# rafaelghiorzi/YOLO-MS

Hardware: AMD Instinct MI355X
Metric: images/sec (train+infer) YOLO-MS-S 640x640 bf16 at 1/2/4/8 MI355X; mAP parity (higher is better)
Workload: dtype bf16; 1 GPU; configs[2]: YOLO-MS-S (reference YOLOv8-'s' graph) 640x640 bf16 training, B=64/GPU, fwd+loss+bwd+SGD-nesterov step; global_batch=64, per_gpu_batch=64, img=640, parallelism=dp1, hip_graph=False

## Files before the change

include/yms.h:

```cpp
#ifndef YMS_H
#define YMS_H

#include <stddef.h>
#include <stdint.h>

#ifdef __cplusplus
extern "C" {
#endif

typedef int yms_status;
#define YMS_OK 0
#define YMS_ERR_INVALID 1
#define YMS_ERR_UNSUPPORTED 2
#define YMS_ERR_LAUNCH 3

#define YMS_F32 0
#define YMS_BF16 1
#define YMS_F16 2

#define YMS_ACT_NONE 0
#define YMS_ACT_SILU 1

typedef struct {
  int n, h, w, cin, cout, k, stride, pad, ho, wo, dtype;
// ... 56 lines not shown
  yms_conv_shape shape;
  const void* dz; int dz_ld, dz_off;
  const void* wpacked_t;
  void* dx; int dx_ld, dx_off;
  int accumulate;
} yms_conv_dgrad_job;
yms_status yms_conv_fwd_group(int njobs, const yms_conv_fwd_job* jobs, void* stream);
yms_status yms_conv_dgrad_group(int njobs, const yms_conv_dgrad_job* jobs, void* stream);
int yms_conv_fwd_group_launches(int njobs, const yms_conv_fwd_job* jobs);
int yms_conv_dgrad_group_launches(int njobs, const yms_conv_dgrad_job* jobs);
size_t yms_conv_wgrad_ws_bytes(const yms_conv_shape* s);
yms_status yms_conv_wgrad(const yms_conv_shape* s, const void* x, int x_ld, int x_off,
                          const void* dz, int dz_ld, int dz_off, float* ws, size_t ws_bytes,
                          float* dw, int accumulate, void* stream);

yms_status yms_bn_fold(int c, const float* gamma, const float* beta, const float* rmean,
                       const float* rvar, float eps, float* scale, float* shift, void* stream);
yms_status yms_bn_finalize(int c, float* stats, int rows, int stats_ld, long count,
                           const float* gamma, const float* beta, float* rmean, float* rvar,
                           float momentum, float eps, float* mean_invstd, float* scale,
                           float* shift, void* stream);
yms_status yms_bn_finalize_ld(int c, float* stats, int rows, int stats_ld, long count,
                              const float* gamma, const float* beta, float* rmean, float* rvar,
                              float momentum, float eps, float* mean_invstd, int mi_ld, float* scale,
                              float* shift, void* stream);
yms_status yms_affine_act(int dtype, long npix, int c, const void* z, int z_ld, int z_off,
                          const float* scale, const float* shift, int act,
                          const void* res, int res_ld, int res_off,
                          void* y, int y_ld, int y_off, void* stream);
int yms_bn_bwd_rows(long npix, int c);
yms_status yms_bn_act_bwd_reduce(int dtype, long npix, int c, const void* z, int z_ld, int z_off,
                                 const void* gy, int gy_ld, int gy_off, const float* scale,
                                 const float* shift, const float* mean_invstd, int act,
                                 float* ws, void* stream);
yms_status yms_bn_act_bwd_finalize(int c, const float* ws, int rows, long count,
                                   float* dgamma, float* dbeta, float* coef, void* stream);
yms_status yms_bn_act_bwd_apply(int dtype, long npix, int c, const void* z, int z_ld, int z_off,
                                const void* gy, int gy_ld, int gy_off, const float* scale,
                                const float* shift, const float* mean_invstd, const float* coef,
                                int act, void* dz, int dz_ld, int dz_off,
                                void* gres, int gres_ld, int gres_off, int gres_acc, void* stream);
yms_status yms_bn_act_bwd_reduce_finalize(int dtype, long npix, int c, const void* z, int z_ld, int z_off,
                                          const void* gy, int gy_ld, int gy_off, const float* scale,
                                          const float* shift, const float* mean_invstd, int act, float* ws,
                                          unsigned* counter, float* dgamma, float* dbeta, float* coef,
                                          void* stream);
yms_status yms_bias_bwd(int dtype, long npix, int c, const void* gy, int gy_ld, int gy_off,
                        float* ws, unsigned* counter, float* dbias, void* stream);
typedef struct {
  int c;
  float* stats; int rows, stats_ld; long count;
  const float* gamma; const float* beta; float* rmean; float* rvar;
  float momentum, eps;
  float* mean_invstd; int mi_ld;
  float* scale; float* shift;
} yms_bn_finalize_job;
typedef struct {
  long npix; int c;
  const void* z; int z_ld, z_off;
  const void* gy; int gy_ld, gy_off;
  const float* scale; const float* shift; const float* mean_invstd; const float* coef;
  int act;
  void* out; int out_ld, out_off;
  void* res; int res_ld, res_off, res_acc;
  float* ws; unsigned* counter; float* dbias;
} yms_bn_pass_job;
typedef struct {
  int c;
  const float* ws; int rows; long count;
  float* dgamma; float* dbeta; float* coef;
} yms_bn_bwd_finalize_job;
yms_status yms_bn_finalize_group(int njobs, const yms_bn_finalize_job* jobs, void* stream);
yms_status yms_affine_act_group(int dtype, int njobs, const yms_bn_pass_job* jobs, void* stream);
yms_status yms_bn_act_bwd_reduce_group(int dtype, int njobs, const yms_bn_pass_job* jobs, void* stream);
yms_status yms_bn_act_bwd_finalize_group(int njobs, const yms_bn_bwd_finalize_job* jobs, void* stream);
yms_status yms_bn_act_bwd_apply_group(int dtype, int njobs, const yms_bn_pass_job* jobs, void* stream);
yms_status yms_bias_bwd_group(int dtype, int njobs, const yms_bn_pass_job* jobs, void* stream);

yms_status yms_sppf_pool_fwd(int dtype, int n, int h, int w, int c, void* buf, int ld, int off,
                             void* stream);
size_t yms_sppf_ws_bytes(int n, int h, int w, int c);
yms_status yms_sppf_pool_bwd(int dtype, int n, int h, int w, int c, const void* buf, int ld,
                             int off, void* gbuf, int gld, int goff, void* ws, void* stream);
yms_status yms_upsample2x_fwd(int dtype, int n, int h, int w, int c, const void* x, int x_ld,
                              int x_off, void* y, int y_ld, int y_off, void* stream);
yms_status yms_upsample2x_bwd(int dtype, int n, int h, int w, int c, const void* gy, int gy_ld,
                              int gy_off, void* gx, int gx_ld, int gx_off, int accumulate,
                              void* stream);
yms_status yms_pack_input(int dtype, int n, int c, int h, int w, const float* x, void* y, int ld,
                          void* stream);
yms_status yms_nhwc_to_nchw(int dtype, int dtype_nchw, int n, int h, int w, int c, const void* x,
                            int ld, int off, void* y, void* stream);
yms_status yms_nchw_to_nhwc(int dtype_nchw, int dtype, int n, int h, int w, int c, const void* x,
                            void* y, int ld, int off, int accumulate, void* stream);
yms_status yms_zero(void* p, size_t bytes, void* stream);
yms_status yms_copy(void* dst, const void* src, size_t bytes, void* stream);
yms_status yms_cast(int dtype_in, int dtype_out, long count, const void* x, void* y, void* stream);

typedef struct {
  int n, h, w, c, k, dtype;
} yms_dw_shape;
int yms_dwconv_stats_rows(const yms_dw_shape* s);
yms_status yms_dwconv_fwd(const yms_dw_shape* s, const void* x, int x_ld, int x_off, const float* w, void* y,
                          int y_ld, int y_off, const float* scale, const float* shift, int act, float* stats,
                          int stats_ld, void* stream);
yms_status yms_dwconv_dgrad(const yms_dw_shape* s, const void* dz, int dz_ld, int dz_off, const float* w, void* dx,
                            int dx_ld, int dx_off, int accumulate, void* stream);
size_t yms_dwconv_wgrad_ws_bytes(const yms_dw_shape* s);
yms_status yms_dwconv_wgrad(const yms_dw_shape* s, const void* x, int x_ld, int x_off, const void* dz, int dz_ld,
                            int dz_off, float* ws, size_t ws_bytes, float* dw, int accumulate, void* stream);
yms_status yms_add_views(int dtype, long npix, int c, const void* a, int a_ld, int a_off, const void* b, int b_ld,
                         int b_off, void* y, int y_ld, int y_off, int accumulate, void* stream);
yms_status yms_add_grad2(int dtype, long npix, int c, const void* g, int g_ld, int g_off, void* ga, int ga_ld,
                         int ga_off, int acc1, void* gb, int gb_ld, int gb_off, int acc2, void* stream);

yms_status yms_map_match(int n_images, const float* det_boxes, const float* det_scores, const int* det_labels,
                         const int* det_off, const float* gt_boxes, const int* gt_labels, const int* gt_off,
                         uint8_t* tp, uint8_t* kept, int* rank_ws, int max_gt_per_image, void* stream);
yms_status yms_map_accumulate(int n_det, const float* scores, const int* labels, const int* image,
                              const uint8_t* tp, const uint8_t* kept, int n_classes, const int* n_gt,
                              double* ap, double* map);
yms_status yms_map_match_coco(int n_images, int n_det, const float* det_boxes, const float* det_scores,
                              const int* det_labels, const int* det_off, const float* gt_boxes, const int* gt_labels,
                              const int* gt_off, int n_thr, const double* iou_thrs, uint16_t* matched,
                              uint16_t* ignored, uint8_t* gt_ignore, int* rank_ws, int max_gt_per_image,
                              void* stream);
yms_status yms_map_accumulate_coco(int n_det, const float* scores, const int* labels, const int* image,
                                   const int* rank, const uint16_t* matched, const uint16_t* ignored, int n_thr,
                                   int n_classes, const int* npig, double* precision, double* recall);

yms_status yms_resize_normalize(int dtype, int n, const void* images, int out_h, int out_w, const float* mean,
                                const float* std, void* out, void* stream);
size_t yms_augment_image_bytes(void);
yms_status yms_augment_normalize(int dtype, int n, const void* images, int out_h, int out_w, const float* mean,
                                 const float* std, void* out, void* stream);
size_t yms_mosaic_image_bytes(void);
yms_status yms_mosaic_normalize(int dtype, int n, const void* records, int out_h, int out_w, const float* mean,
                                const float* std, void* out, void* stream);

size_t yms_det_loss_ws_bytes(int batch, int anchors, int nc, int n_targets);
yms_status yms_det_loss(int dtype, int batch, int nc, int nlevels, const void* const* maps, void* const* grads,
                        const int* hs, const int* ws_, const float* strides, int ld, const float* targets,
                        int n_targets, float img_w, float img_h, int iou_type, const float* pos_weight,
                        const float* lambdas, void* ws, size_t ws_bytes, float* out, void* stream);
yms_status yms_scale_by_device_scalar(int dtype, int nbuf, void* const* bufs, const long* counts, const float* g,
                                      void* stream);

yms_status yms_head_decode(int dtype, int n, int nc, int nlev, const void* const* lvl,
                           const int* hs, const int* ws, int no_ld, const float* strides,
                           float* out, float conf, float* boxes_xyxy, float* nms_score,
                           int* label, void* stream);
yms_status yms_dfl(int dtype, int n, int A, int ch, const void* x, void* out, void* stream);
yms_status yms_nms_prep(int n, int A, int nc, const float* pred, float conf, float* boxes_xyxy,
                        float* score, int* label, void* stream);
size_t yms_nms_ws_bytes(int n, int A, int nc);
size_t yms_nms_ws_bytes_min(int n, int A, int nc);
yms_status yms_nms_classwise(int n, int A, int nc, const float* boxes_xyxy, const float* score,
                             const int* label, double iou, int64_t* keep_idx, int* keep_lbl,
                             int* counts, void* ws, size_t ws_bytes, void* stream);
yms_status yms_nms_single(int m, const float* boxes, const float* scores, double iou,
                          int64_t* keep, int* count, void* ws, size_t ws_bytes, void* stream);

#ifdef __cplusplus
}
#endif
#endif
// ... 1 lines not shown
```

yolo-ms_amd/csrc/bn_pool.hip:

```cpp
#include <cstdlib>
#include <algorithm>
#include <vector>

#include "yms_common.hpp"

namespace yms {

static inline unsigned grid_for(long items, int block = 256, long cap = 16384) {
  long g = (items + block - 1) / block;
  if (g < 1) g = 1;
  return (unsigned)std::min(g, cap);
}

__global__ void bn_fold_kernel(int c, const float* g, const float* b, const float* rm,
                               const float* rv, float eps, float* scale, float* shift) {
  const int i = blockIdx.x * blockDim.x + threadIdx.x;
  if (i >= c) return;
  if (!g) {
    scale[i] = 1.0f;
    shift[i] = b ? b[i] : 0.0f;
    return;
  }
  const float sc = g[i] / sqrtf(rv[i] + eps);
  scale[i] = sc;
// ... 720 lines not shown
      }
    }
    Vec8<T>::store(buf + (long)pix * ld + out_off + g * 8, m);
  }
}

template <typename T>
__global__ void pool5_argmax_kernel(int n, int h, int w, int c, const T* buf, int ld, int in_off,
                                    uint8_t* arg) {
  const int G = (c + 7) >> 3;
  const uint32_t total = (uint32_t)n * h * w * G;
  for (uint32_t t = blockIdx.x * blockDim.x + threadIdx.x; t < total; t += gridDim.x * blockDim.x) {
    const int g = (int)(t % G);
    uint32_t r = t / G;
    const int x = (int)(r % w);
    r /= w;
    const int y = (int)(r % h);
    const int b = (int)(r / h);
    const int c0 = g * 8, nv = min(8, c - c0);
    float best[8];
    uint8_t idx[8];
#pragma unroll
    for (int i = 0; i < 8; ++i) { best[i] = -INFINITY; idx[i] = 255; }
    for (int ky = 0; ky < 5; ++ky) {
      const int yy = y - 2 + ky;
      if (yy < 0 || yy >= h) continue;
      for (int kx = 0; kx < 5; ++kx) {
        const int xx = x - 2 + kx;
        if (xx < 0 || xx >= w) continue;
        float v[8];
        load8(buf + (((long)b * h + yy) * w + xx) * ld + in_off + c0, nv, v);
#pragma unroll
        for (int i = 0; i < 8; ++i)
          if (idx[i] == 255 || v[i] > best[i] || v[i] != v[i]) {
            best[i] = v[i];
            idx[i] = (uint8_t)(ky * 5 + kx);
          }
      }
    }
    uint8_t* a = arg + ((((long)b * h + y) * w + x) * G + g) * 8;
#pragma unroll
    for (int i = 0; i < 8; ++i) a[i] = idx[i];
  }
}

template <typename T>
__global__ void pool5_gather_kernel(int n, int h, int w, int c, const uint8_t* arg, T* g, int ld,
                                    int in_off, int out_off) {
  const int G = (c + 7) >> 3;
  const uint32_t total = (uint32_t)n * h * w * G;
  for (uint32_t t = blockIdx.x * blockDim.x + threadIdx.x; t < total; t += gridDim.x * blockDim.x) {
    const int gg = (int)(t % G);
    uint32_t r = t / G;
    const int x = (int)(r % w);
    r /= w;
    const int y = (int)(r % h);
    const int b = (int)(r / h);
    const int c0 = gg * 8, nv = min(8, c - c0);
    float acc[8];
    load8(g + (((long)b * h + y) * w + x) * ld + in_off + c0, nv, acc);
    for (int ky = 0; ky < 5; ++ky) {
      const int oy = y - ky + 2;
      if (oy < 0 || oy >= h) continue;
      for (int kx = 0; kx < 5; ++kx) {
        const int ox = x - kx + 2;
        if (ox < 0 || ox >= w) continue;
        const long o = ((long)b * h + oy) * w + ox;
        const uint8_t* a = arg + (o * G + gg) * 8;
        const uint2 av = *reinterpret_cast<const uint2*>(a);
        const uint8_t want = (uint8_t)(ky * 5 + kx);
        float gv[8];
        load8(g + o * ld + out_off + c0, nv, gv);
#pragma unroll
        for (int i = 0; i < 8; ++i) {
          const uint8_t ai = (uint8_t)(((i < 4 ? av.x : av.y) >> (8 * (i & 3))) & 0xff);
          if (ai == want) acc[i] += gv[i];
        }
      }
    }
    store8(g + (((long)b * h + y) * w + x) * ld + in_off + c0, nv, acc);
  }
}


template <typename T>
__global__ void upsample_fwd_kernel(int n, int h, int w, int c, const T* x, int x_ld, int x_off,
                                    T* y, int y_ld, int y_off) {
  const int G = (c + 7) >> 3;
  const int H2 = 2 * h, W2 = 2 * w;
  const long total = (long)n * H2 * W2 * G;
  for (long t = blockIdx.x * (long)blockDim.x + threadIdx.x; t < total; t += (long)gridDim.x * blockDim.x) {
    const int g = (int)(t % G);
    long r = t / G;
    const int X = (int)(r % W2);
    r /= W2;
    const int Y = (int)(r % H2);
    const int b = (int)(r / H2);
    const int c0 = g * 8, nv = min(8, c - c0);
    float v[8];
    load8(x + (((long)b * h + (Y >> 1)) * w + (X >> 1)) * x_ld + x_off + c0, nv, v);
    store8(y + (((long)b * H2 + Y) * W2 + X) * y_ld + y_off + c0, nv, v);
  }
}

template <typename T>
__global__ void upsample_bwd_kernel(int n, int h, int w, int c, const T* gy, int gy_ld, int gy_off,
                                    T* gx, int gx_ld, int gx_off, int accumulate) {
  const int G = (c + 7) >> 3;
  const int W2 = 2 * w;
  const long total = (long)n * h * w * G;
  for (long t = blockIdx.x * (long)blockDim.x + threadIdx.x; t < total; t += (long)gridDim.x * blockDim.x) {
    const int g = (int)(t % G);
    long r = t / G;
    const int x = (int)(r % w);
    r /= w;
    const int y = (int)(r % h);
    const int b = (int)(r / h);
    const int c0 = g * 8, nv = min(8, c - c0);
    float s[8];
    T* dst = gx + (((long)b * h + y) * w + x) * gx_ld + gx_off + c0;
    if (accumulate) load8(dst, nv, s);
    else {
#pragma unroll
      for (int i = 0; i < 8; ++i) s[i] = 0.f;
    }
#pragma unroll
    for (int d = 0; d < 4; ++d) {
      float v[8];
      const int Y = 2 * y + (d >> 1), X = 2 * x + (d & 1);
      load8(gy + (((long)b * 2 * h + Y) * W2 + X) * gy_ld + gy_off + c0, nv, v);
#pragma unroll
      for (int i = 0; i < 8; ++i) s[i] += v[i];
    }
    store8(dst, nv, s);
  }
}

template <typename T>
__global__ void pack_input_kernel(int n, int c, int h, int w, const float* x, T* y, int ld) {
  const long npix = (long)n * h * w;
  const long hw = (long)h * w;
  for (long t = blockIdx.x * (long)blockDim.x + threadIdx.x; t < npix; t += (long)gridDim.x * blockDim.x) {
    const long b = t / hw, s = t - b * hw;
    for (int c0 = 0; c0 < ld; c0 += 8) {
      float v[8];
#pragma unroll
      for (int i = 0; i < 8; ++i) v[i] = (c0 + i < c) ? x[(b * c + c0 + i) * hw + s] : 0.0f;
      Vec8<T>::store(y + t * ld + c0, v);
    }
  }
}

template <typename TI, typename TO>
__global__ void nhwc_to_nchw_kernel(int n, long hw, int c, const TI* x, int ld, int off, TO* y) {
  __shared__ float tile[64][65];
  const long pt = (long)blockIdx.x * 64;
  const int ct = blockIdx.y * 64;
  const int b = blockIdx.z;
  const int tx = threadIdx.x & 63, ty = threadIdx.x >> 6;
  for (int r = ty; r < 64; r += 4) {
    const long p = pt + r;
    const int ch = ct + tx;
    tile[r][tx] = (p < hw && ch < c) ? (float)x[((long)b * hw + p) * ld + off + ch] : 0.f;
  }
  __syncthreads();
  for (int r = ty; r < 64; r += 4) {
// ... 319 lines not shown
                            mean_invstd, c, scale, shift, stream);
}

yms_status yms_affine_act(int dtype, long npix, int c, const void* z, int z_ld, int z_off,
                          const float* scale, const float* shift, int act,
                          const void* res, int res_ld, int res_off,
                          void* y, int y_ld, int y_off, void* stream) {
  const yms_bn_pass_job j{npix, c, z, z_ld, z_off, nullptr, 0, 0, scale, shift, nullptr, nullptr, act, y, y_ld, y_off,
                          (void*)res, res_ld, res_off};
  return run_pass<AffinePass>(dtype, 1, &j, stream);
}

int yms_bn_bwd_rows(long npix, int c) {
  if (npix <= 0 || c <= 0) return 0;
  return (int)pix_blocks(npix, bwd_pix_per_block(npix, c, false));
}

yms_status yms_bn_act_bwd_reduce(int dtype, long npix, int c, const void* z, int z_ld, int z_off,
                                 const void* gy, int gy_ld, int gy_off, const float* scale,
                                 const float* shift, const float* mean_invstd, int act,
                                 float* ws, void* stream) {
  const yms_bn_pass_job j{npix, c, z, z_ld, z_off, gy, gy_ld, gy_off, scale, shift, mean_invstd, nullptr, act,
                          nullptr, 0, 0, nullptr, 0, 0, 0, ws};
  return run_pass<ReducePass>(dtype, 1, &j, stream);
}

yms_status yms_bn_act_bwd_finalize(int c, const float* ws, int rows, long count, float* dgamma,
                                   float* dbeta, float* coef, void* stream) {
  const yms_bn_bwd_finalize_job j{c, ws, rows, count, dgamma, dbeta, coef};
  return run_pass<BwdFinalizePass>(0, 1, &j, stream);
}

yms_status yms_bn_act_bwd_apply(int dtype, long npix, int c, const void* z, int z_ld, int z_off,
                                const void* gy, int gy_ld, int gy_off, const float* scale,
                                const float* shift, const float* mean_invstd, const float* coef,
                                int act, void* dz, int dz_ld, int dz_off,
                                void* gres, int gres_ld, int gres_off, int gres_acc, void* stream) {
  const yms_bn_pass_job j{npix, c, z, z_ld, z_off, gy, gy_ld, gy_off, scale, shift, mean_invstd, coef, act,
                          dz, dz_ld, dz_off, gres, gres_ld, gres_off, gres_acc};
  return run_pass<ApplyPass>(dtype, 1, &j, stream);
}

yms_status yms_bn_act_bwd_reduce_finalize(int dtype, long npix, int c, const void* z, int z_ld, int z_off,
                                          const void* gy, int gy_ld, int gy_off, const float* scale,
                                          const float* shift, const float* mean_invstd, int act, float* ws,
                                          unsigned* counter, float* dgamma, float* dbeta, float* coef,
                                          void* stream) {
  const yms_bn_pass_job j{npix, c, z, z_ld, z_off, gy, gy_ld, gy_off, scale, shift, mean_invstd, nullptr, act,
                          nullptr, 0, 0, nullptr, 0, 0, 0, ws, counter};
  if (yms_status e = reduce_check(j, z != nullptr, true)) return e;
  return launch_reduce_finalize(dtype, j, z != nullptr, BwdFin{counter, dgamma, dbeta, coef, npix}, (hipStream_t)stream);
}

yms_status yms_bias_bwd(int dtype, long npix, int c, const void* gy, int gy_ld, int gy_off,
                        float* ws, unsigned* counter, float* dbias, void* stream) {
  const yms_bn_pass_job j{npix, c, nullptr, 0, 0, gy, gy_ld, gy_off, nullptr, nullptr, nullptr, nullptr, YMS_ACT_NONE,
                          nullptr, 0, 0, nullptr, 0, 0, 0, ws, counter, dbias};
  return run_pass<BiasPass>(dtype, 1, &j, stream);
}

yms_status yms_bn_finalize_group(int njobs, const yms_bn_finalize_job* jobs, void* stream) {
  return run_pass<FinalizePass>(0, njobs, jobs, stream);
}
yms_status yms_affine_act_group(int dtype, int njobs, const yms_bn_pass_job* jobs, void* stream) {
  return run_pass<AffinePass>(dtype, njobs, jobs, stream);
}
yms_status yms_bn_act_bwd_reduce_group(int dtype, int njobs, const yms_bn_pass_job* jobs, void* stream) {
  return run_pass<ReducePass>(dtype, njobs, jobs, stream);
}
yms_status yms_bn_act_bwd_finalize_group(int njobs, const yms_bn_bwd_finalize_job* jobs, void* stream) {
  return run_pass<BwdFinalizePass>(0, njobs, jobs, stream);
}
yms_status yms_bn_act_bwd_apply_group(int dtype, int njobs, const yms_bn_pass_job* jobs, void* stream) {
  return run_pass<ApplyPass>(dtype, njobs, jobs, stream);
}
yms_status yms_bias_bwd_group(int dtype, int njobs, const yms_bn_pass_job* jobs, void* stream) {
  return run_pass<BiasPass>(dtype, njobs, jobs, stream);
}

size_t yms_sppf_ws_bytes(int n, int h, int w, int c) {
  return (size_t)n * h * w * ((c + 7) / 8) * 8;
}

yms_status yms_sppf_pool_fwd(int dtype, int n, int h, int w, int c, void* buf, int ld, int off,
                             void* stream) {
  if (n <= 0 || h <= 0 || w <= 0 || !buf || !vok(ld, off, 4 * c) || c % 8 != 0) return YMS_ERR_INVALID;
  const long items = (long)n * h * w * ((c + 7) / 8);
  if (items >= (1l << 31)) return YMS_ERR_UNSUPPORTED;
  for (int k = 1; k <= 3; ++k)
    YMS_DT_DISPATCH(dtype, T, hipLaunchKernelGGL(pool5_fwd_kernel<T>, dim3(grid_for(items)), dim3(256), 0,
                                                 (hipStream_t)stream, n, h, w, c, (T*)buf, ld,
                                                 off + (k - 1) * c, off + k * c));
  return launch_status();
}

yms_status yms_sppf_pool_bwd(int dtype, int n, int h, int w, int c, const void* buf, int ld,
                             int off, void* gbuf, int gld, int goff, void* ws, void* stream) {
  if (n <= 0 || !buf || !gbuf || !ws || !vok(ld, off, 4 * c) || !vok(gld, goff, 4 * c) || c % 8 != 0)
    return YMS_ERR_INVALID;
  if (ld != gld) return YMS_ERR_UNSUPPORTED;
  const long items = (long)n * h * w * ((c + 7) / 8);
  if (items >= (1l << 31)) return YMS_ERR_UNSUPPORTED;
  hipStream_t st = (hipStream_t)stream;
  for (int k = 3; k >= 1; --k) {
    YMS_DT_DISPATCH(dtype, T, {
      hipLaunchKernelGGL(pool5_argmax_kernel<T>, dim3(grid_for(items)), dim3(256), 0, st, n, h, w, c,
                         (const T*)buf, ld, off + (k - 1) * c, (uint8_t*)ws);
      hipLaunchKernelGGL(pool5_gather_kernel<T>, dim3(grid_for(items)), dim3(256), 0, st, n, h, w, c,
                         (const uint8_t*)ws, (T*)gbuf, gld, goff + (k - 1) * c, goff + k * c);
    });
  }
  return launch_status();
}

yms_status yms_upsample2x_fwd(int dtype, int n, int h, int w, int c, const void* x, int x_ld,
                              int x_off, void* y, int y_ld, int y_off, void* stream) {
  if (n <= 0 || !x || !y || !vok(x_ld, x_off, c) || !vok(y_ld, y_off, c)) return YMS_ERR_INVALID;
  const long items = (long)n * 4 * h * w * ((c + 7) / 8);
  YMS_DT_DISPATCH(dtype, T, hipLaunchKernelGGL(upsample_fwd_kernel<T>, dim3(grid_for(items)), dim3(256), 0,
                                               (hipStream_t)stream, n, h, w, c, (const T*)x, x_ld, x_off,
                                               (T*)y, y_ld, y_off));
  return launch_status();
}

yms_status yms_upsample2x_bwd(int dtype, int n, int h, int w, int c, const void* gy, int gy_ld,
                              int gy_off, void* gx, int gx_ld, int gx_off, int accumulate,
                              void* stream) {
  if (n <= 0 || !gy || !gx || !vok(gy_ld, gy_off, c) || !vok(gx_ld, gx_off, c)) return YMS_ERR_INVALID;
  const long items = (long)n * h * w * ((c + 7) / 8);
  YMS_DT_DISPATCH(dtype, T, hipLaunchKernelGGL(upsample_bwd_kernel<T>, dim3(grid_for(items)), dim3(256), 0,
                                               (hipStream_t)stream, n, h, w, c, (const T*)gy, gy_ld, gy_off,
                                               (T*)gx, gx_ld, gx_off, accumulate));
  return launch_status();
}

yms_status yms_pack_input(int dtype, int n, int c, int h, int w, const float* x, void* y, int ld,
                          void* stream) {
  if (n <= 0 || c <= 0 || !x || !y || ld % 8 != 0 || ld < c) return YMS_ERR_INVALID;
  const long npix = (long)n * h * w;
  YMS_DT_DISPATCH(dtype, T, hipLaunchKernelGGL(pack_input_kernel<T>, dim3(grid_for(npix)), dim3(256), 0,
                                               (hipStream_t)stream, n, c, h, w, x, (T*)y, ld));
  return launch_status();
}

#define YMS_DT2(d1, d2, T1, T2, ...)                                          \
  YMS_DT_DISPATCH(d1, T1, { YMS_DT_DISPATCH(d2, T2, __VA_ARGS__); })

yms_status yms_nhwc_to_nchw(int dtype, int dtype_nchw, int n, int h, int w, int c, const void* x,
                            int ld, int off, void* y, void* stream) {
  if (n <= 0 || h <= 0 || w <= 0 || !x || !y || !vok(ld, off, c)) return YMS_ERR_INVALID;
  const long hw = (long)h * w;
  dim3 grid((unsigned)cdiv(hw, 64), (unsigned)cdiv(c, 64), (unsigned)n);
  YMS_DT2(dtype, dtype_nchw, TI, TO, hipLaunchKernelGGL((nhwc_to_nchw_kernel<TI, TO>), grid, dim3(256), 0,
                                                        (hipStream_t)stream, n, hw, c, (const TI*)x, ld, off,
                                                        (TO*)y));
  return launch_status();
}

yms_status yms_nchw_to_nhwc(int dtype_nchw, int dtype, int n, int h, int w, int c, const void* x,
                            void* y, int ld, int off, int accumulate, void* stream) {
  if (n <= 0 || h <= 0 || w <= 0 || !x || !y || !vok(ld, off, c)) return YMS_ERR_INVALID;
  const long hw = (long)h * w;
  dim3 grid((unsigned)cdiv(hw, 64), (unsigned)cdiv(c, 64), (unsigned)n);
  YMS_DT2(dtype_nchw, dtype, TI, TO, hipLaunchKernelGGL((nchw_to_nhwc_kernel<TI, TO>), grid, dim3(256), 0,
                                                        (hipStream_t)stream, n, hw, c, (const TI*)x, (TO*)y,
                                                        ld, off, accumulate));
  return launch_status();
}

yms_status yms_cast(int dtype_in, int dtype_out, long count, const void* x, void* y, void* stream) {
  if (count <= 0 || !x || !y) return YMS_ERR_INVALID;
  YMS_DT2(dtype_in, dtype_out, TI, TO, hipLaunchKernelGGL((cast_kernel<TI, TO>), dim3(grid_for(count)),
                                                          dim3(256), 0, (hipStream_t)stream, count,
                                                          (const TI*)x, (TO*)y));
  return launch_status();
}

}

extern "C" yms_status yms_zero(void* p, size_t bytes, void* stream) {
  if (!p) return YMS_ERR_INVALID;
  if (bytes == 0) return YMS_OK;
  return hipMemsetAsync(p, 0, bytes, (hipStream_t)stream) == hipSuccess ? YMS_OK : YMS_ERR_LAUNCH;
}

extern "C" yms_status yms_copy(void* dst, const void* src, size_t bytes, void* stream) {
// ... 6 lines not shown
```

yolo-ms_amd/yms/_lib.py:

```python
from __future__ import annotations

import ctypes
import operator
import os
import types

import torch

_HERE = os.path.dirname(os.path.abspath(__file__))
LIB_PATH = os.environ.get("YMS_LIB") or os.path.join(_HERE, "libyms.so")

F32, BF16, F16 = 0, 1, 2
ACT_NONE, ACT_SILU = 0, 1

_DT = {torch.float32: F32, torch.bfloat16: BF16, torch.float16: F16}


def dtype_code(dt):
    try:
        return _DT[dt]
    except KeyError:
        raise RuntimeError(f"yms: unsupported dtype {dt}; use float32, bfloat16 or float16") from None


# ... 17 lines not shown


def _fields(spec):
    t = {"p": ctypes.c_void_p, "i": ctypes.c_int, "l": ctypes.c_long, "f": ctypes.c_float, "s": ConvShape}
    return [(n, t[k]) for n, k in (f.split(":") for f in spec.split())]


class ConvFwdJob(ctypes.Structure):
    _fields_ = _fields("shape:s x:p x_ld:i x_off:i wpacked:p y:p y_ld:i y_off:i scale:p shift:p act:i "
                       "res:p res_ld:i res_off:i stats:p")


class ConvDgradJob(ctypes.Structure):
    _fields_ = _fields("shape:s dz:p dz_ld:i dz_off:i wpacked_t:p dx:p dx_ld:i dx_off:i accumulate:i")


class BnFinalizeJob(ctypes.Structure):
    _fields_ = _fields("c:i stats:p rows:i stats_ld:i count:l gamma:p beta:p rmean:p rvar:p momentum:f eps:f "
                       "mean_invstd:p mi_ld:i scale:p shift:p")


class BnPassJob(ctypes.Structure):
    _fields_ = _fields("npix:l c:i z:p z_ld:i z_off:i gy:p gy_ld:i gy_off:i scale:p shift:p mean_invstd:p coef:p "
                       "act:i out:p out_ld:i out_off:i res:p res_ld:i res_off:i res_acc:i ws:p counter:p dbias:p")


class BnBwdFinalizeJob(ctypes.Structure):
    _fields_ = _fields("c:i ws:p rows:i count:l dgamma:p dbeta:p coef:p")


_L = ctypes.c_long
_F = ctypes.c_float
_D = ctypes.c_double
_SZ = ctypes.c_size_t
_SP = ctypes.POINTER(ConvShape)
_DP = ctypes.POINTER(DwShape)

_SIGS = {
    "yms_version": (ctypes.c_char_p, []),
    "yms_status_string": (ctypes.c_char_p, [_I]),
    "yms_conv_packed_elems": (_SZ, [_SP, _I]),
    "yms_conv_pack_weight": (_I, [_SP, _P, _P, _I, _P]),
    "yms_pack_job_init": (_I, [_SP, _P, _P, _I, ctypes.POINTER(PackJob)]),
    "yms_conv_pack_weights_batched": (_I, [_I, _P, _P, _P]),
    "yms_conv_stats_rows": (_I, [_SP]),
    "yms_conv_stats_ld": (_I, [_SP]),
    "yms_conv_direct_set": (_I, [_I]),
    "yms_conv_fwd": (_I, [_SP, _P, _I, _I, _P, _P, _I, _I, _P, _P, _I, _P, _I, _I, _P, _P]),
    "yms_conv_stem_supported": (_I, [_SP]),
    "yms_conv_stem_stats_rows": (_I, [_SP]),
    "yms_conv_stem_fwd": (_I, [_SP, _P, _P, _P, _I, _I, _P, _P, _I, _P, _I, _P]),
    "yms_conv_stem_wgrad_ws_bytes": (_SZ, [_SP]),
    "yms_conv_stem_wgrad": (_I, [_SP, _P, _P, _I, _I, _P, _I, _I, _P, _P, _P, _P, _I, _P, _SZ, _P, _I, _P]),
    "yms_conv_dgrad": (_I, [_SP, _P, _I, _I, _P, _P, _I, _I, _I, _P]),
    "yms_conv_dgrad_bnred_rows": (_I, [_SP]),
    "yms_conv_dgrad_bnred": (_I, [_SP, _P, _I, _I, _P, _P, _I, _I, _I, _P, _I, _I, _P, _P, _P, _I, _P, _P]),
    "yms_conv_fwd_group": (_I, [_I, _P, _P]),
    "yms_conv_dgrad_group": (_I, [_I, _P, _P]),
    "yms_conv_fwd_group_launches": (_I, [_I, _P]),
    "yms_conv_dgrad_group_launches": (_I, [_I, _P]),
    "yms_conv_wgrad_ws_bytes": (_SZ, [_SP]),
    "yms_conv_wgrad": (_I, [_SP, _P, _I, _I, _P, _I, _I, _P, _SZ, _P, _I, _P]),
    "yms_bn_fold": (_I, [_I, _P, _P, _P, _P, _F, _P, _P, _P]),
    "yms_bn_finalize": (_I, [_I, _P, _I, _I, _L, _P, _P, _P, _P, _F, _F, _P, _P, _P, _P]),
    "yms_bn_finalize_ld": (_I, [_I, _P, _I, _I, _L, _P, _P, _P, _P, _F, _F, _P, _I, _P, _P, _P]),
    "yms_affine_act": (_I, [_I, _L, _I, _P, _I, _I, _P, _P, _I, _P, _I, _I, _P, _I, _I, _P]),
    "yms_bn_bwd_rows": (_I, [_L, _I]),
    "yms_bn_act_bwd_reduce": (_I, [_I, _L, _I, _P, _I, _I, _P, _I, _I, _P, _P, _P, _I, _P, _P]),
    "yms_bn_act_bwd_finalize": (_I, [_I, _P, _I, _L, _P, _P, _P, _P]),
    "yms_bn_act_bwd_apply": (_I, [_I, _L, _I, _P, _I, _I, _P, _I, _I, _P, _P, _P, _P, _I, _P, _I, _I,
                                  _P, _I, _I, _I, _P]),
    "yms_bn_act_bwd_reduce_finalize": (_I, [_I, _L, _I, _P, _I, _I, _P, _I, _I, _P, _P, _P, _I, _P, _P, _P, _P,
                                            _P, _P]),
    "yms_bias_bwd": (_I, [_I, _L, _I, _P, _I, _I, _P, _P, _P, _P]),
    "yms_bn_finalize_group": (_I, [_I, _P, _P]),
    "yms_affine_act_group": (_I, [_I, _I, _P, _P]),
    "yms_bn_act_bwd_reduce_group": (_I, [_I, _I, _P, _P]),
    "yms_bn_act_bwd_finalize_group": (_I, [_I, _P, _P]),
    "yms_bn_act_bwd_apply_group": (_I, [_I, _I, _P, _P]),
    "yms_bias_bwd_group": (_I, [_I, _I, _P, _P]),
    "yms_sppf_ws_bytes": (_SZ, [_I, _I, _I, _I]),
    "yms_sppf_pool_fwd": (_I, [_I, _I, _I, _I, _I, _P, _I, _I, _P]),
    "yms_sppf_pool_bwd": (_I, [_I, _I, _I, _I, _I, _P, _I, _I, _P, _I, _I, _P, _P]),
    "yms_upsample2x_fwd": (_I, [_I, _I, _I, _I, _I, _P, _I, _I, _P, _I, _I, _P]),
    "yms_upsample2x_bwd": (_I, [_I, _I, _I, _I, _I, _P, _I, _I, _P, _I, _I, _I, _P]),
    "yms_pack_input": (_I, [_I, _I, _I, _I, _I, _P, _P, _I, _P]),
    "yms_nhwc_to_nchw": (_I, [_I, _I, _I, _I, _I, _I, _P, _I, _I, _P, _P]),
    "yms_nchw_to_nhwc": (_I, [_I, _I, _I, _I, _I, _I, _P, _P, _I, _I, _I, _P]),
    "yms_cast": (_I, [_I, _I, _L, _P, _P, _P]),
    "yms_zero": (_I, [_P, _SZ, _P]),
    "yms_copy": (_I, [_P, _P, _SZ, _P]),
    "yms_dwconv_stats_rows": (_I, [_DP]),
    "yms_dwconv_fwd": (_I, [_DP, _P, _I, _I, _P, _P, _I, _I, _P, _P, _I, _P, _I, _P]),
    "yms_dwconv_dgrad": (_I, [_DP, _P, _I, _I, _P, _P, _I, _I, _I, _P]),
    "yms_dwconv_wgrad_ws_bytes": (_SZ, [_DP]),
    "yms_dwconv_wgrad": (_I, [_DP, _P, _I, _I, _P, _I, _I, _P, _SZ, _P, _I, _P]),
    "yms_add_views": (_I, [_I, _L, _I, _P, _I, _I, _P, _I, _I, _P, _I, _I, _I, _P]),
    "yms_add_grad2": (_I, [_I, _L, _I, _P, _I, _I, _P, _I, _I, _I, _P, _I, _I, _I, _P]),
    "yms_map_match": (_I, [_I, _P, _P, _P, _P, _P, _P, _P, _P, _P, _P, _I, _P]),
    "yms_map_accumulate": (_I, [_I, _P, _P, _P, _P, _P, _I, _P, _P, _P]),
    "yms_map_match_coco": (_I, [_I, _I, _P, _P, _P, _P, _P, _P, _P, _I, _P, _P, _P, _P, _P, _I, _P]),
    "yms_map_accumulate_coco": (_I, [_I, _P, _P, _P, _P, _P, _P, _I, _I, _P, _P, _P]),
    "yms_det_loss_ws_bytes": (_SZ, [_I, _I, _I, _I]),
    "yms_stream_create_cu_subset": (_I, [_I, _I, ctypes.POINTER(ctypes.c_void_p)]),
    "yms_resize_normalize": (_I, [_I, _I, _P, _I, _I, _P, _P, _P, _P]),
    "yms_augment_image_bytes": (_SZ, []),
    "yms_augment_normalize": (_I, [_I, _I, _P, _I, _I, _P, _P, _P, _P]),
    "yms_mosaic_image_bytes": (_SZ, []),
    "yms_mosaic_normalize": (_I, [_I, _I, _P, _I, _I, _P, _P, _P, _P]),
    "yms_det_loss": (_I, [_I, _I, _I, _I, _P, _P, _P, _P, _P, _I, _P, _I, _F, _F, _I, _P, _P, _P, _SZ, _P, _P]),
    "yms_scale_by_device_scalar": (_I, [_I, _I, _P, _P, _P, _P]),
    "yms_head_decode": (_I, [_I, _I, _I, _I, _P, _P, _P, _I, _P, _P, _F, _P, _P, _P, _P]),
    "yms_dfl": (_I, [_I, _I, _I, _I, _P, _P, _P]),
    "yms_nms_prep": (_I, [_I, _I, _I, _P, _F, _P, _P, _P, _P]),
    "yms_nms_ws_bytes": (_SZ, [_I, _I, _I]),
    "yms_nms_ws_bytes_min": (_SZ, [_I, _I, _I]),
    "yms_nms_classwise": (_I, [_I, _I, _I, _P, _P, _P, _D, _P, _P, _P, _P, _SZ, _P]),
    "yms_nms_single": (_I, [_I, _P, _P, _D, _P, _P, _P, _SZ, _P]),
}

EXPORTED = tuple(_SIGS)
_lib = None


def lib():
    global _lib
    if _lib is None:
        if not os.path.exists(LIB_PATH):
            raise RuntimeError(
                f"yms: HIP library {LIB_PATH} not found -- build it with "
                "`python -c 'import __graft_entry__ as g; g.build()'` (make -C yolo-ms_amd/csrc)")
        L = ctypes.CDLL(LIB_PATH)
        for name, (res, args) in _SIGS.items():
            fn = getattr(L, name)
            fn.restype = res
            fn.argtypes = args
        _lib = L
    return _lib


def check(status, what):
    if status != 0:
        msg = lib().yms_status_string(status).decode()
        raise RuntimeError(f"yms: {what} failed: {msg} (status {status})")


_prof = None
_CONV = ("yms_conv_fwd", "yms_conv_dgrad", "yms_conv_dgrad_bnred", "yms_conv_wgrad", "yms_conv_stem_fwd")
_DW = ("yms_dwconv_fwd", "yms_dwconv_dgrad", "yms_dwconv_wgrad")
_GROUP_AS = {"yms_conv_fwd_group": "yms_conv_fwd", "yms_conv_dgrad_group": "yms_conv_dgrad",
             "yms_affine_act_group": "yms_affine_act", "yms_bn_act_bwd_reduce_group": "yms_bn_act_bwd_reduce",
             "yms_bn_act_bwd_apply_group": "yms_bn_act_bwd_apply", "yms_bn_finalize_group": "yms_bn_finalize",
             "yms_bn_act_bwd_finalize_group": "yms_bn_act_bwd_finalize", "yms_bias_bwd_group": "yms_bias_bwd"}
_HOST_ONLY = {"yms_map_accumulate", "yms_map_accumulate_coco", "yms_pack_job_init", "yms_conv_fwd_group_launches",
              "yms_conv_dgrad_group_launches"}
_STREAM_LAST = {n for n, (res, args) in _SIGS.items()
                if res is _I and args and args[-1] is _P and n not in _HOST_ONLY}


_FN = {}


def _elt(dt):
    return 4 if dt == F32 else 2


# ... 113 lines not shown
```

Before: 3851 images/sec.

## Fuse SPPF three-pool chain into single LDS-resident kernels for fwd and bwd

Adds fused SPPF kernels that keep one image's 8-channel plane in LDS and run all three cascaded 5x5 max pools (forward), or the argmax and gradient scatter chain (backward), in a single launch using separable row/column passes. This replaces three pool launches forward and the multiple argmax/scatter launches backward, which removes intermediate global round trips and launch overhead for small spatial maps (20x20 at 640 input). The fused path is used by default for bf16/f16 when the plane fits the LDS and thread budget. The cost is serialized per-block work and __syncthreads barriers, plus lower occupancy from dynamic LDS.

Measured after the change: 3913 images/sec (median of 6 runs). 1.02x the previous value.

```diff
diff --git a/include/yms.h b/include/yms.h
--- a/include/yms.h
+++ b/include/yms.h
@@ -162,6 +162,8 @@
 size_t yms_sppf_ws_bytes(int n, int h, int w, int c);
 yms_status yms_sppf_pool_bwd(int dtype, int n, int h, int w, int c, const void* buf, int ld,
                              int off, void* gbuf, int gld, int goff, void* ws, void* stream);
+int yms_sppf_fused_fits(int dtype, int h, int w, int c);
+int yms_sppf_route_set(int v);
 yms_status yms_upsample2x_fwd(int dtype, int n, int h, int w, int c, const void* x, int x_ld,
                               int x_off, void* y, int y_ld, int y_off, void* stream);
 yms_status yms_upsample2x_bwd(int dtype, int n, int h, int w, int c, const void* gy, int gy_ld,
diff --git a/yolo-ms_amd/csrc/bn_pool.hip b/yolo-ms_amd/csrc/bn_pool.hip
--- a/yolo-ms_amd/csrc/bn_pool.hip
+++ b/yolo-ms_amd/csrc/bn_pool.hip
@@ -826,6 +826,233 @@
   }
 }
 
+constexpr int SPPF_NP = 3;
+constexpr int SPPF_BWD_BPP = 56;
+constexpr int SPPF_LDS_MAX = 32 * 1024;
+
+template <typename T>
+__device__ __forceinline__ u32x4 sppf_pack(const float (&v)[8]) {
+  T t[8];
+#pragma unroll
+  for (int i = 0; i < 8; ++i) t[i] = (T)v[i];
+  u32x4 r;
+  __builtin_memcpy(&r, t, sizeof(r));
+  return r;
+}
+template <typename T>
+__device__ __forceinline__ void sppf_unpack(const u32x4& r, float (&v)[8]) {
+  Raw8<T> q;
+  q.v[0] = r;
+  unpack8<T>(q, v);
+}
+__device__ __forceinline__ bool sppf_block(int nlog, int G, int& b, int& g) {
+  const int l = (int)((blockIdx.x & 7) * (gridDim.x >> 3) + (blockIdx.x >> 3));
+  if (l >= nlog) return false;
+  g = l % G;
+  b = l / G;
+  return true;
+}
+
+template <typename T>
+__global__ __launch_bounds__(256) void sppf_chain_fwd_kernel(int nlog, int h, int w, int c, T* buf, int ld, int off) {
+  static_assert(sizeof(T) == 2, "16-bit planes");
+  extern __shared__ u32x4 sppf_lds[];
+  int b, g;
+  if (!sppf_block(nlog, c >> 3, b, g)) return;
+  const int P = h * w;
+  u32x4* X = sppf_lds;
+  u32x4* R = sppf_lds + P;
+  T* base = buf + (long)b * P * ld + off + g * 8;
+  int py[SPPF_NP], px[SPPF_NP];
+#pragma unroll
+  for (int i = 0; i < SPPF_NP; ++i) {
+    const int p = threadIdx.x + 256 * i;
+    py[i] = p / w;
+    px[i] = p - py[i] * w;
+    if (p < P) X[p] = *reinterpret_cast<const u32x4*>(base + (long)p * ld);
+  }
+  __syncthreads();
+  for (int k = 1; k <= 3; ++k) {
+#pragma unroll
+    for (int i = 0; i < SPPF_NP; ++i) {
+      const int p = threadIdx.x + 256 * i;
+      if (p >= P) continue;
+      float m[8];
+#pragma unroll
+      for (int j = 0; j < 8; ++j) m[j] = -INFINITY;
+      const int x0 = max(px[i] - 2, 0), x1 = min(px[i] + 2, w - 1);
+      for (int q = p - px[i] + x0; q <= p - px[i] + x1; ++q) {
+        float v[8];
+        sppf_unpack<T>(X[q], v);
+#pragma unroll
+        for (int j = 0; j < 8; ++j) m[j] = (v[j] > m[j] || v[j] != v[j]) ? v[j] : m[j];
+      }
+      R[p] = sppf_pack<T>(m);
+    }
+    __syncthreads();
+#pragma unroll
+    for (int i = 0; i < SPPF_NP; ++i) {
+      const int p = threadIdx.x + 256 * i;
+      if (p >= P) continue;
+      float m[8];
+#pragma unroll
+      for (int j = 0; j < 8; ++j) m[j] = -INFINITY;
+      const int y0 = max(py[i] - 2, 0), y1 = min(py[i] + 2, h - 1);
+      for (int yy = y0; yy <= y1; ++yy) {
+        float v[8];
+        sppf_unpack<T>(R[yy * w + px[i]], v);
+#pragma unroll
+        for (int j = 0; j < 8; ++j) m[j] = (v[j] > m[j] || v[j] != v[j]) ? v[j] : m[j];
+      }
+      const u32x4 r = sppf_pack<T>(m);
+      X[p] = r;
+      *reinterpret_cast<u32x4*>(base + (long)p * ld + k * c) = r;
+    }
+    __syncthreads();
+  }
+}
+
+template <typename T>
+__global__ __launch_bounds__(256) void sppf_chain_bwd_kernel(int nlog, int h, int w, int c, const T* buf, int ld,
+                                                             int off, T* gbuf, int gld, int goff) {
+  static_assert(sizeof(T) == 2, "16-bit planes");
+  extern __shared__ u32x4 sppf_lds[];
+  int b, g;
+  if (!sppf_block(nlog, c >> 3, b, g)) return;
+  const int P = h * w;
+  u32x4* V = sppf_lds;
+  uint2* A = reinterpret_cast<uint2*>(sppf_lds);
+  u32x4* GI = sppf_lds + P;
+  u32x4* GO = sppf_lds + 2 * P;
+  uint2* RK = reinterpret_cast<uint2*>(sppf_lds + 3 * P);
+  const T* vbase = buf + (long)b * P * ld + off + g * 8;
+  T* gbase = gbuf + (long)b * P * gld + goff + g * 8;
+  u32x4 vreg[SPPF_NP], greg[SPPF_NP];
+#pragma unroll
+  for (int i = 0; i < SPPF_NP; ++i) {
+    const int p = threadIdx.x + 256 * i;
+    vreg[i] = greg[i] = u32x4{0u, 0u, 0u, 0u};
+    if (p < P) {
+      vreg[i] = *reinterpret_cast<const u32x4*>(vbase + (long)p * ld + 2 * c);
+      greg[i] = *reinterpret_cast<const u32x4*>(gbase + (long)p * gld + 2 * c);
+      GI[p] = *reinterpret_cast<const u32x4*>(gbase + (long)p * gld + 3 * c);
+    }
+  }
+  for (int k = 3; k >= 1; --k) {
+#pragma unroll
+    for (int i = 0; i < SPPF_NP; ++i) {
+      const int p = threadIdx.x + 256 * i;
+      if (p < P) V[p] = vreg[i];
+    }
+    __syncthreads();
+#pragma unroll 1
+    for (int p = threadIdx.x; p < P; p += 256) {
+      const int px = p % w;
+      const int kx0 = max(2 - px, 0), kx1 = min(w + 1 - px, 4);
+      float best[8];
+      uint32_t idx[8];
+      sppf_unpack<T>(V[p - 2 + kx0], best);
+#pragma unroll
+      for (int j = 0; j < 8; ++j) idx[j] = (uint32_t)kx0;
+      for (int kx = kx0 + 1; kx <= kx1; ++kx) {
+        float v[8];
+        sppf_unpack<T>(V[p - 2 + kx], v);
+#pragma unroll
+        for (int j = 0; j < 8; ++j) {
+          const bool t = v[j] > best[j] || v[j] != v[j];
+          best[j] = t ? v[j] : best[j];
+          idx[j] = t ? (uint32_t)kx : idx[j];
+        }
+      }
+      GO[p] = sppf_pack<T>(best);
+      RK[p] = make_uint2(idx[0] | idx[1] << 8 | idx[2] << 16 | idx[3] << 24,
+                         idx[4] | idx[5] << 8 | idx[6] << 16 | idx[7] << 24);
+    }
+    __syncthreads();
+#pragma unroll 1
+    for (int p = threadIdx.x; p < P; p += 256) {
+      const int py = p / w;
+      const int ky0 = max(2 - py, 0), ky1 = min(h + 1 - py, 4);
+      float best[8];
+      uint32_t idx[8];
+      {
+        const int q = p + (ky0 - 2) * w;
+        sppf_unpack<T>(GO[q], best);
+        const uint2 rk = RK[q];
+        const uint32_t a = 5u * ky0 * 0x01010101u;
+#pragma unroll
+        for (int j = 0; j < 8; ++j) idx[j] = (j < 4 ? rk.x : rk.y) + a;
+      }
+      for (int ky = ky0 + 1; ky <= ky1; ++ky) {
+        const int q = p + (ky - 2) * w;
+        float v[8];
+        sppf_unpack<T>(GO[q], v);
+        const uint2 rk = RK[q];
+        const uint32_t a = 5u * ky * 0x01010101u;
+        const uint32_t cx = rk.x + a, cy = rk.y + a;
+#pragma unroll
+        for (int j = 0; j < 8; ++j) {
+          const bool t = v[j] > best[j] || v[j] != v[j];
+          best[j] = t ? v[j] : best[j];
+          idx[j] = t ? (j < 4 ? cx : cy) : idx[j];
+        }
+      }
+      uint2 a = make_uint2(0u, 0u);
+#pragma unroll
+      for (int j = 0; j < 4; ++j) {
+        a.x |= idx[j] & (0xffu << (8 * j));
+        a.y |= idx[4 + j] & (0xffu << (8 * j));
+      }
+      A[p] = a;
+    }
+    __syncthreads();
+#pragma unroll
+    for (int i = 0; i < SPPF_NP; ++i) {
+      const int p = threadIdx.x + 256 * i;
+      if (p < P) GO[p] = greg[i];
+    }
+    if (k > 1) {
+#pragma unroll
+      for (int i = 0; i < SPPF_NP; ++i) {
+        const int p = threadIdx.x + 256 * i;
+        if (p < P) {
+          vreg[i] = *reinterpret_cast<const u32x4*>(vbase + (long)p * ld + (k - 2) * c);
+          greg[i] = *reinterpret_cast<const u32x4*>(gbase + (long)p * gld + (k - 2) * c);
+        }
+      }
+    }
+#pragma unroll 1
+    for (int p = threadIdx.x; p < P; p += 256) {
+      const int py = p / w, px = p - py * w;
+      float acc[8];
+      sppf_unpack<T>(GO[p], acc);
+      const int ky0 = max(py + 3 - h, 0), ky1 = min(py + 2, 4);
+      const int kx0 = max(px + 3 - w, 0), kx1 = min(px + 2, 4);
+      for (int ky = ky0; ky <= ky1; ++ky) {
+        for (int kx = kx0; kx <= kx1; ++kx) {
+          const int o = p + (2 - ky) * w + 2 - kx;
+          const uint2 av = A[o];
+          float gv[8];
+          sppf_unpack<T>(GI[o], gv);
+          const uint32_t want = (uint32_t)(ky * 5 + kx);
+#pragma unroll
+          for (int j = 0; j < 8; ++j) {
+            const uint32_t aj = ((j < 4 ? av.x : av.y) >> (8 * (j & 3))) & 0xffu;
+            if (aj == want) acc[j] += gv[j];
+          }
+        }
+      }
+      const u32x4 r = sppf_pack<T>(acc);
+      *reinterpret_cast<u32x4*>(gbase + (long)p * gld + (k - 1) * c) = r;
+      GO[p] = r;
+    }
+    __syncthreads();
+    u32x4* t = GI;
+    GI = GO;
+    GO = t;
+  }
+}
+
 
 template <typename T>
 __global__ void upsample_fwd_kernel(int n, int h, int w, int c, const T* x, int x_ld, int x_off,
@@ -1311,11 +1538,39 @@
   return (size_t)n * h * w * ((c + 7) / 8) * 8;
 }
 
+int yms_sppf_fused_fits(int dtype, int h, int w, int c) {
+  if (dtype != YMS_BF16 && dtype != YMS_F16) return 0;
+  if (h <= 0 || w <= 0 || c <= 0 || c % 8 != 0) return 0;
+  const long p = (long)h * w;
+  return p * SPPF_BWD_BPP <= SPPF_LDS_MAX && p <= 256 * SPPF_NP;
+}
+static int& sppf_route() {
+  static int r = 1;
+  return r;
+}
+int yms_sppf_route_set(int v) {
+  const int prev = sppf_route();
+  if (v >= 0) sppf_route() = v ? 1 : 0;
+  return prev;
+}
+
 yms_status yms_sppf_pool_fwd(int dtype, int n, int h, int w, int c, void* buf, int ld, int off,
                              void* stream) {
   if (n <= 0 || h <= 0 || w <= 0 || !buf || !vok(ld, off, 4 * c) || c % 8 != 0) return YMS_ERR_INVALID;
   const long items = (long)n * h * w * ((c + 7) / 8);
   if (items >= (1l << 31)) return YMS_ERR_UNSUPPORTED;
+  if (sppf_route() && yms_sppf_fused_fits(dtype, h, w, c)) {
+    const int nlog = n * (c / 8);
+    const dim3 grid((unsigned)rup(nlog, 8));
+    const size_t lds = (size_t)h * w * 32;
+    if (dtype == YMS_BF16)
+      hipLaunchKernelGGL(sppf_chain_fwd_kernel<bf16>, grid, dim3(256), lds, (hipStream_t)stream, nlog, h, w, c,
+                         (bf16*)buf, ld, off);
+    else
+      hipLaunchKernelGGL(sppf_chain_fwd_kernel<f16>, grid, dim3(256), lds, (hipStream_t)stream, nlog, h, w, c,
+                         (f16*)buf, ld, off);
+    return launch_status();
+  }
   for (int k = 1; k <= 3; ++k)
     YMS_DT_DISPATCH(dtype, T, hipLaunchKernelGGL(pool5_fwd_kernel<T>, dim3(grid_for(items)), dim3(256), 0,
                                                  (hipStream_t)stream, n, h, w, c, (T*)buf, ld,
@@ -1331,6 +1586,18 @@
   const long items = (long)n * h * w * ((c + 7) / 8);
   if (items >= (1l << 31)) return YMS_ERR_UNSUPPORTED;
   hipStream_t st = (hipStream_t)stream;
+  if (sppf_route() && yms_sppf_fused_fits(dtype, h, w, c)) {
+    const int nlog = n * (c / 8);
+    const dim3 grid((unsigned)rup(nlog, 8));
+    const size_t lds = (size_t)h * w * SPPF_BWD_BPP;
+    if (dtype == YMS_BF16)
+      hipLaunchKernelGGL(sppf_chain_bwd_kernel<bf16>, grid, dim3(256), lds, st, nlog, h, w, c, (const bf16*)buf, ld,
+                         off, (bf16*)gbuf, gld, goff);
+    else
+      hipLaunchKernelGGL(sppf_chain_bwd_kernel<f16>, grid, dim3(256), lds, st, nlog, h, w, c, (const f16*)buf, ld,
+                         off, (f16*)gbuf, gld, goff);
+    return launch_status();
+  }
   for (int k = 3; k >= 1; --k) {
     YMS_DT_DISPATCH(dtype, T, {
       hipLaunchKernelGGL(pool5_argmax_kernel<T>, dim3(grid_for(items)), dim3(256), 0, st, n, h, w, c,
diff --git a/yolo-ms_amd/yms/_lib.py b/yolo-ms_amd/yms/_lib.py
--- a/yolo-ms_amd/yms/_lib.py
+++ b/yolo-ms_amd/yms/_lib.py
@@ -123,6 +123,8 @@
     "yms_sppf_ws_bytes": (_SZ, [_I, _I, _I, _I]),
     "yms_sppf_pool_fwd": (_I, [_I, _I, _I, _I, _I, _P, _I, _I, _P]),
     "yms_sppf_pool_bwd": (_I, [_I, _I, _I, _I, _I, _P, _I, _I, _P, _I, _I, _P, _P]),
+    "yms_sppf_fused_fits": (_I, [_I, _I, _I, _I]),
+    "yms_sppf_route_set": (_I, [_I]),
     "yms_upsample2x_fwd": (_I, [_I, _I, _I, _I, _I, _P, _I, _I, _P, _I, _I, _P]),
     "yms_upsample2x_bwd": (_I, [_I, _I, _I, _I, _I, _P, _I, _I, _P, _I, _I, _I, _P]),
     "yms_pack_input": (_I, [_I, _I, _I, _I, _I, _P, _P, _I, _P]),
```
